# plumer/pbrs

Measured on AMD Instinct MI355X. Metric: Msamples/s, higher is better.
Workload: dtype f32

## Files before the change

### pbrs_amd/csrc/device/traverse.h

```cpp
#pragma once
#include "shapes.h"

#include "probes.h"

struct RaySpace {
    f3 o, d;
    f3 nr;
    bool fast;
};
PD uint32_t dir_in_range(float x) {
    uint32_t e = (pn_bits(x) >> 23) & 0xffu;
    return (e - (127u - 40u) <= 80u) ? 1u : 0u;
}
PD uint32_t origin_in_range(float x) {
    uint32_t u = pn_bits(x) & 0x7fffffffu;
    uint32_t e = u >> 23;
    return ((u == 0u) | (e - (127u - 60u) <= 100u)) ? 1u : 0u;
}
PD RaySpace make_space(f3 o, f3 d, bool scene_ok) {
    RaySpace r;
    r.o = o;
    r.d = d;
    r.fast = ((scene_ok ? 1u : 0u) & dir_in_range(d.x) & dir_in_range(d.y) & dir_in_range(d.z) & origin_in_range(o.x) &
              origin_in_range(o.y) & origin_in_range(o.z)) != 0u;
    r.nr = gray(0.0f);
    if (r.fast) r.nr = mk3(-(1.0f / d.x), -(1.0f / d.y), -(1.0f / d.z));
    return r;
}
PD RaySpace reload_world(const DevScene& S, LaneStack stk) {
    const float4 a = stk.ro[stk.item], b = stk.rd[stk.item];
    return make_space(mk3(a.x, a.y, a.z), mk3(b.x, b.y, b.z), S.fast_slab != 0);
}
#define PBRS_SPACE_WORLD 0u
#define PBRS_SPACE_MOVED 1u
#define PBRS_SPACE_TRANSLATED 2u
PD void leave_instance(const DevScene& S, LaneStack stk, uint32_t moved, RaySpace& C) {
    if (moved == PBRS_SPACE_TRANSLATED && C.fast) {
        const float4 a = stk.ro[stk.item];
        C.o = mk3(a.x, a.y, a.z);
    } else if (moved != PBRS_SPACE_WORLD) {
        C = reload_world(S, stk);
    }
}
PD float qdiv(float nn, float d, float nr) {
    const float q0 = nn * nr;
    const float e = __builtin_fmaf(d, q0, nn);
    return __builtin_fmaf(e, nr, q0);
}
PD bool slab_rs(const pbrs_node& n, const RaySpace& R, float t_max) {
    if (!R.fast) return slab_test(nmin(n), nmax(n), R.o, R.d, t_max);
    float t0x = qdiv(R.o.x - n.min[0], R.d.x, R.nr.x), t0y = qdiv(R.o.y - n.min[1], R.d.y, R.nr.y), t0z = qdiv(R.o.z - n.min[2], R.d.z, R.nr.z);
    float t1x = qdiv(R.o.x - n.max[0], R.d.x, R.nr.x), t1y = qdiv(R.o.y - n.max[1], R.d.y, R.nr.y), t1z = qdiv(R.o.z - n.max[2], R.d.z, R.nr.z);
    float lo_el = __builtin_fmaxf(__builtin_fmaxf(__builtin_fminf(t0x, t1x), __builtin_fminf(t0y, t1y)), __builtin_fminf(t0z, t1z));
    float hi_el = __builtin_fminf(__builtin_fminf(__builtin_fmaxf(t0x, t1x), __builtin_fmaxf(t0y, t1y)), __builtin_fmaxf(t0z, t1z));
    float t_low = __builtin_fmaxf(lo_el, 0.0f);
    float t_high = __builtin_fminf(hi_el, t_max);
    return t_low <= t_high;
}
#include "wide.h"

struct InstHead {
    uint32_t flags, blas_root, mesh_flags, wide_root;
};
static_assert(offsetof(pbrs_instance, flags) == 108 && offsetof(pbrs_instance, blas_root) == 112 && offsetof(pbrs_instance, mesh_flags) == 116 &&
                  offsetof(pbrs_instance, pad) == 120 && sizeof(pbrs_instance) == 128 && alignof(pbrs_instance) <= 16,
              "pbrs_instance layout (load_inst_head, wide root in pad[1], shading class in pad[0])");
static_assert(sizeof(pbrs_node) == 32 && offsetof(pbrs_node, a) == 12 && offsetof(pbrs_node, max) == 16 && offsetof(pbrs_node, b) == 28, "pbrs_node layout (load_node)");
static_assert(sizeof(pbrs_wnode) == 128 && offsetof(pbrs_wnode, hi) == 48 && offsetof(pbrs_wnode, child) == 96, "pbrs_wnode layout (wide_test)");
static_assert(sizeof(pbrs_tri_verts) == 48, "pbrs_tri_verts layout (load_tri)");
PD InstHead load_inst_head(const pbrs_instance& in) {
    uint32_t f = in.flags;
    uint4 r = *reinterpret_cast<const uint4*>(&in.blas_root);
    asm volatile("" : "+v"(f), "+v"(r.x), "+v"(r.y), "+v"(r.w));
    return {f, r.x, r.y, r.w};
}
PD uint32_t enter_instance(const DevScene& S, const pbrs_instance& in, uint32_t in_flags, RaySpace& C, bool need_slab, LaneStack stk) {
    if ((in_flags & PBRS_INSTANCE_IDENTITY) && C.fast && C.o.x != 0.0f && C.o.y != 0.0f && C.o.z != 0.0f) return PBRS_SPACE_WORLD;
    f3 oo = xf_apply(in.inv, C.o, 1.0f);
    if (need_slab && (in_flags & PBRS_INSTANCE_TRANSLATION) && C.fast) {
        C.o = oo;
        if (!(origin_in_range(oo.x) & origin_in_range(oo.y) & origin_in_range(oo.z))) {
            C.fast = false;
            C.nr = gray(0.0f);
        }
        return PBRS_SPACE_TRANSLATED;
    }
    f3 od = xf_apply(in.inv, C.d, 0.0f);
    if (need_slab) {
        C = make_space(oo, od, S.fast_slab != 0);
    } else {
        C.o = oo;
        C.d = od;
        C.fast = false;
    }
    return PBRS_SPACE_MOVED;
}

#ifndef PBRS_EARLY_OUT
#define PBRS_EARLY_OUT 1
#endif
#define PBRS_WALK_IDLE 0u
#define PBRS_WALK_NODE 1u
#define PBRS_WALK_LEAF 2u
#define PBRS_WALK_DONE 3u
#define PBRS_WALK_SCAN 5u
#define PBRS_WALK_XFER 4u

PD uint32_t lane_prefix(uint64_t mask) {
    return __builtin_amdgcn_mbcnt_hi((uint32_t)(mask >> 32), __builtin_amdgcn_mbcnt_lo((uint32_t)mask, 0u));
}
struct TriShare {
    uint32_t tag;
    uint32_t cnt;
    uint64_t has[4];
    uint32_t off[4];

    PD void build(uint32_t want) {
        const uint32_t lane = threadIdx.x & 63u;
        uint32_t o = 0;
        tag = 0;
        cnt = 0;
#pragma unroll
        for (uint32_t j = 0; j < 4u; ++j) {
            const uint64_t m = __ballot(want > j);
            has[j] = m;
            off[j] = o;
            if (m == 0) continue;
            const uint32_t p = o + lane_prefix(m);
            const bool send = want > j && p < 63u;
            tag |= (uint32_t)__builtin_amdgcn_ds_permute((int)((send ? p : 63u) << 2), send ? (int)(lane | j << 8 | 0x10000u) : 0);
            cnt += send ? 1u : 0u;
            o += (uint32_t)__popcll(m);
        }
    }
    PD bool helper() const { return tag != 0u; }
    PD uint32_t k() const { return (tag >> 8) & 3u; }
    PD uint32_t pos(uint32_t j) const { return off[j] + lane_prefix(has[j]); }
    PD uint32_t from_owner(uint32_t v) const { return (uint32_t)__builtin_amdgcn_ds_bpermute((int)(tag << 2), (int)v); }
    PD float from_owner(float v) const { return __uint_as_float(from_owner(__float_as_uint(v))); }
    PD f3 from_owner(f3 v) const { return mk3(from_owner(v.x), from_owner(v.y), from_owner(v.z)); }
    PD float from_helper(uint32_t at, float v) const {
        return __uint_as_float((uint32_t)__builtin_amdgcn_ds_bpermute((int)(at << 2), (int)__float_as_uint(v)));
    }
};

struct FlatScan {
    PD static uint32_t pull(uint32_t from, uint32_t v) { return (uint32_t)__builtin_amdgcn_ds_bpermute((int)(from << 2), (int)v); }
    PD static float pull(uint32_t from, float v) { return __uint_as_float(pull(from, __float_as_uint(v))); }
    struct Exact {
        RaySpace O;
        float t;
        PD Exact(const RaySpace& R, float t_max) : O(R), t(t_max) {}
        PD Exact from(uint32_t owner) const {
            Exact y = *this;
            y.O.o = mk3(pull(owner, O.o.x), pull(owner, O.o.y), pull(owner, O.o.z));
            y.O.d = mk3(pull(owner, O.d.x), pull(owner, O.d.y), pull(owner, O.d.z));
            y.O.nr = mk3(pull(owner, O.nr.x), pull(owner, O.nr.y), pull(owner, O.nr.z));
            y.O.fast = true;
            y.t = pull(owner, t);
            return y;
        }
        PD bool test(const pbrs_node& n) const { return slab_rs(n, O, t); }
    };
    struct Filter {
        f3 o, r;
        PD Filter(const RaySpace& R, float) : o(R.o), r(-R.nr) {}
        PD Filter from(uint32_t owner) const {
            Filter y = *this;
            y.o = mk3(pull(owner, o.x), pull(owner, o.y), pull(owner, o.z));
            y.r = mk3(pull(owner, r.x), pull(owner, r.y), pull(owner, r.z));
            return y;
        }
        PD bool test(const pbrs_node& n) const {
            return pn_slab_filter(r.x > 0.0f ? n.min[0] : n.max[0], r.y > 0.0f ? n.min[1] : n.max[1], r.z > 0.0f ? n.min[2] : n.max[2],
                                  r.x > 0.0f ? n.max[0] : n.min[0], r.y > 0.0f ? n.max[1] : n.min[1], r.z > 0.0f ? n.max[2] : n.min[2], o.x, o.y, o.z,
                                  r.x, r.y, r.z, pn_inf()) != 0;
        }
    };
    template <class Ray>
    PD static uint32_t scan(const DevScene& S, bool fresh, const RaySpace& R, float t_max, uint32_t& tested) {
        const uint64_t m = __ballot(fresh);
        if (m == 0) return 0u;
// ... 7 lines not shown
        uint32_t mine = 0;
        for (uint32_t base = 0; base < total; base += 64u) {
            const uint32_t p = base + lane;
            const bool valid = p < total;
            const uint32_t r = (p * magic) >> 16, h = p - r * H;
            const Ray O = mine_ray.from(pull(r, list));
            bool pass0 = false, pass1 = false;
            if (valid) {
                pass0 = O.test(load_node(S.nodes + S.flat_off + h));
                tested += 1u;
                if (h + H < S.n_flat) {
                    pass1 = O.test(load_node(S.nodes + S.flat_off + h + H));
                    tested += 1u;
                }
            }
            const uint64_t w0 = __ballot(pass0), w1 = __ballot(pass1);
            const int sft = (int)(rank * H) - (int)base;
            if (fresh && sft > -(int)H && sft < 64) {
                const uint64_t a = sft >= 0 ? w0 >> sft : w0 << -sft, b = sft >= 0 ? w1 >> sft : w1 << -sft;
                const uint32_t keep = (1u << H) - 1u;
                mine |= ((uint32_t)a & keep) | (((uint32_t)b & keep) << H);
            }
        }
        return mine;
    }
    PD static uint32_t run(const DevScene& S, bool fresh, const RaySpace& R, float t_max, uint32_t& tested) { return scan<Exact>(S, fresh, R, t_max, tested); }
    PD static uint32_t run_filter(const DevScene& S, bool fresh, const RaySpace& R, uint32_t& tested) { return scan<Filter>(S, fresh, R, pn_inf(), tested); }
};

template <bool STATS, uint32_t FEAT>
struct ClosestWalk {
    RaySpace C;
    Hit best;
    float t_max, lt, mt, mb1, mb2;
    uint32_t mprim, cur_inst;
    uint32_t inst_info;
    uint32_t leaf_a, leaf_end;
    int sp, blas_base;
    uint32_t cand;
    bool in_blas, moved;
    uint32_t mode;
    static constexpr bool EXT = (FEAT & PBRS_FEAT_EXTENT) != 0u;
    float win;
    bool win_has;
    PBRS_TP_FIELDS

    PD void start(const DevScene& S, f3 o, f3 d, float tmax, LaneStack stk) {
        C = make_space(o, d, S.fast_slab != 0);
        win = 0.0f;
        win_has = false;
        moved = false;
        best.t = pn_inf();
        best.inst = 0xffffffffu;
        best.prim = 0;
        best.b1 = best.b2 = 0.0f;
        in_blas = false;
        t_max = tmax;
        lt = tmax;
        mt = pn_inf();
        mprim = cur_inst = inst_info = leaf_a = leaf_end = 0;
        mb1 = mb2 = 0.0f;
        blas_base = 0;
        cand = 0;
        if ((FEAT & PBRS_FEAT_FLAT_TLAS) && !EXT && S.n_flat != 0u && C.fast) {
            sp = 0;
            mode = PBRS_WALK_SCAN;
        } else {
            stk.put(0, 0u);
            sp = 1;
            mode = PBRS_WALK_NODE;
        }
    }
    PD void scan_wave(const DevScene& S, Cnt<STATS>& cnt) {
        if (!(FEAT & PBRS_FEAT_FLAT_TLAS) || EXT) return;
        uint32_t tested = 0;
        const uint32_t mine = FlatScan::run_filter(S, mode == PBRS_WALK_SCAN, C, tested);
        if (STATS) cnt.c.tlas_nodes += tested;
        if (mode == PBRS_WALK_SCAN) {
            cand = mine;
            mode = PBRS_WALK_NODE;
        }
    }

    PD void node_step(const DevScene& S, LaneStack stk, Cnt<STATS>& cnt) {
        PBRS_TP(0);
        if (in_blas && sp == blas_base) {
            mode = exit_mode();
            return;
        }
        uint32_t ni;
        if (sp == 0) {
            if (!(FEAT & PBRS_FEAT_FLAT_TLAS) || cand == 0u) {
                mode = PBRS_WALK_DONE;
                return;
            }
            ni = S.flat_off + (uint32_t)__builtin_ctz(cand);
            cand &= cand - 1u;
        } else {
            ni = stk.get(--sp);
            if constexpr (EXT) {
                if (!in_blas && (ni & 0x80000000u)) {
                    const bool below_has = (ni & 0x40000000u) != 0u;
                    const float below = __uint_as_float(stk.get(--sp));
                    ni &= 0x3fffffffu;
                    if (win_has) t_max = win;
                    if (below_has && (!win_has || below < win)) win = below;
                    win_has = win_has || below_has;
                    lt = t_max;
                }
            }
            if (STATS) {
                if (in_blas) CNT(blas_nodes);
                else CNT(tlas_nodes);
            }
        }
        const pbrs_node node = walk_node<FEAT>(S, ni);
        PBRS_TP(1);
        if (!slab_rs(node, C, lt)) {
            PBRS_TP(2);
            if (PBRS_EARLY_OUT && in_blas && sp == blas_base) mode = exit_mode();
            return;
        }
        if (!(node.b & PBRS_LEAF_FLAG)) {
            bool left_first = !in_blas || comp(C.d, (int)(node.b & 3u)) > 0.0f;
            uint32_t left = ni + 1, right = node.a;
            if constexpr (EXT) {
                if (!in_blas) {
                    stk.put(sp++, __float_as_uint(win));
                    right |= 0x80000000u | (win_has ? 0x40000000u : 0u);
                    win_has = false;
                }
            }
            stk.put(sp++, left_first ? right : left);
            stk.put(sp++, left_first ? left : right);
            lt = in_blas ? mt : lt;
        } else if (in_blas) {
            PBRS_TP(3);
            PBRS_TP(4);
            leaf_a = node.a;
            leaf_end = node.a + (node.b & ~PBRS_LEAF_FLAG);
            if (leaf_end != leaf_a) mode = PBRS_WALK_LEAF;
            else lt = mt;
        } else {
            cur_inst = node.a;
            inst_info = (node.b >> PBRS_TLAS_LEAF_KIND_SHIFT) & 7u;
            mode = PBRS_WALK_XFER;
        }
    }

    PD void node_step_fast(const DevScene& S, LaneStack stk, Cnt<STATS>& cnt) {
        if constexpr (EXT) return;
        if (sp == (in_blas ? blas_base : 0) || !C.fast) return;
        PBRS_TP(0);
        const uint32_t ni = stk.get(--sp);
        if (STATS) {
            if (in_blas) CNT(blas_nodes);
            else CNT(tlas_nodes);
        }
        const pbrs_node node = walk_node<FEAT>(S, ni);
        PBRS_TP(1);
        RaySpace F = C;
        F.fast = true;
        if (!slab_rs(node, F, lt)) {
            PBRS_TP(2);
            return;
        }
        if (!(node.b & PBRS_LEAF_FLAG)) {
            bool left_first = !in_blas || comp(C.d, (int)(node.b & 3u)) > 0.0f;
            uint32_t left = ni + 1, right = node.a;
            stk.put(sp++, left_first ? right : left);
            stk.put(sp++, left_first ? left : right);
            lt = in_blas ? mt : lt;
        } else if (in_blas) {
            PBRS_TP(3);
            PBRS_TP(4);
            leaf_a = node.a;
            leaf_end = node.a + (node.b & ~PBRS_LEAF_FLAG);
            if (leaf_end != leaf_a) mode = PBRS_WALK_LEAF;
            else lt = mt;
        } else {
            cur_inst = node.a;
            inst_info = (node.b >> PBRS_TLAS_LEAF_KIND_SHIFT) & 7u;
            mode = PBRS_WALK_XFER;
        }
    }

    PD void meet_best(Cnt<STATS>& cnt) {
        if (mt < pn_inf() || (inst_info & 0x80000000u)) {
            CNT(instance_hits);
            if constexpr (EXT) {
                if (!win_has || !(win < mt)) win = mt;
                win_has = true;
            }
            if (!(best.t < mt)) {
                best.t = mt;
                best.inst = cur_inst;
                best.prim = mprim;
                best.b1 = mb1;
                best.b2 = mb2;
                if constexpr (!EXT) t_max = mt;
            }
        }
    }
    PD uint32_t exit_mode() const {
        const bool nothing_above = blas_base == 0 && (!(FEAT & PBRS_FEAT_FLAT_TLAS) || cand == 0u);
        return nothing_above ? PBRS_WALK_DONE : PBRS_WALK_XFER;
    }
    PD void finish(Cnt<STATS>& cnt) {
        if (in_blas) {
            in_blas = false;
            meet_best(cnt);
        }
    }
    PD void xfer_step(const DevScene& S, LaneStack stk, Cnt<STATS>& cnt) {
        mode = PBRS_WALK_NODE;
        if (in_blas) {
            PBRS_TP(7);
            in_blas = false;
            leave_instance(S, stk, !moved ? PBRS_SPACE_WORLD : (inst_info & 0x40000000u) ? PBRS_SPACE_TRANSLATED : PBRS_SPACE_MOVED, C);
            meet_best(cnt);
            lt = t_max;
            return;
        }
        const pbrs_instance& in = S.inst[cur_inst];
        CNT(instances);
        PBRS_TP(6);
        const uint32_t kind = inst_info;
        if ((FEAT & PBRS_FEAT_ANALYTIC) && kind != PBRS_SHAPE_MESH && kind != PBRS_SHAPE_TRIANGLE) {
            analytic_visit(S, in, kind, cnt);
            return;
        }
        const InstHead H = load_inst_head(in);
        const uint32_t space = enter_instance(S, in, H.flags, C, kind == PBRS_SHAPE_MESH, stk);
        moved = space != PBRS_SPACE_WORLD;
        in_blas = true;
        blas_base = sp;
        lt = t_max;
        mt = pn_inf();
        if (kind == PBRS_SHAPE_MESH) {
            inst_info = kind | (H.mesh_flags << 3) | (space == PBRS_SPACE_TRANSLATED ? 0x40000000u : 0u);
            stk.put(sp++, H.blas_root);
        } else if (kind == PBRS_SHAPE_TRIANGLE) {
            inst_info = kind | (PBRS_MESH_SHADING_OK_MASK << 3);
            leaf_a = H.blas_root;
            leaf_end = H.blas_root + 1u;
            mode = PBRS_WALK_LEAF;
        }
    }

    PD void analytic_visit(const DevScene& S, const pbrs_instance& in, uint32_t kind, Cnt<STATS>& cnt) {
        if (!(FEAT & PBRS_FEAT_ANALYTIC)) return;
        const f3 o = xf_apply(in.inv, C.o, 1.0f), d = xf_apply(in.inv, C.d, 0.0f);
        const float ext = t_max;
        const float* p = S.shapes[in.shape_index].p;
// ... 505 lines not shown
```

### pbrs_amd/csrc/host/scene_prepare.cpp

```cpp
#include "scene_prepare.h"

#include <algorithm>
#include <cstring>
#include <map>
#include <string>

#include "../../../include/pbrs_numeric.h"
#include "../../../include/pbrs_scene_spec.h"

namespace pbrs {
namespace {

SceneCheck refuse(int code, const char* message) { return SceneCheck{code, message, SceneLevels{}}; }

void tree_heights(const pbrs_node* nodes, uint32_t n, std::vector<uint32_t>& h) {
    h.assign(n, 1u);
    for (uint32_t i = n; i-- > 0;)
        if (!(nodes[i].b & PBRS_LEAF_FLAG)) h[i] = std::max(h[i + 1], h[nodes[i].a]) + 1u;
}

SceneLevels scene_levels(const pbrs_scene_desc& d) {
    SceneLevels l;
    std::vector<uint32_t> th, bh;
    tree_heights(d.tlas_nodes, d.n_tlas_nodes, th);
    tree_heights(d.blas_nodes, d.n_blas_nodes, bh);
    l.tlas = th[0];
    for (uint32_t i = 0; i < d.n_meshes; ++i) l.max_blas = std::max(l.max_blas, bh[d.meshes[i].root]);
    for (uint32_t i = 0; i < d.n_instances; ++i)
        if (d.instances[i].shape_kind == PBRS_SHAPE_MESH) l.max_blas = std::max(l.max_blas, bh[d.instances[i].blas_root]);
    l.stack = std::max(l.tlas, l.tlas - 1u + l.max_blas);
    bool has_quad = false, has_mesh = false;
    for (uint32_t i = 0; i < d.n_instances; ++i) {
        has_quad = has_quad || d.instances[i].shape_kind == PBRS_SHAPE_QUAD;
        has_mesh = has_mesh || d.instances[i].shape_kind == PBRS_SHAPE_MESH;
    }
    l.exact_extent = has_quad && has_mesh;
    if (l.exact_extent) l.stack += l.tlas + 1u;
    return l;
}

bool tlas_scanned(const pbrs_scene_desc& d) { return d.n_instances >= PBRS_FLAT_TLAS_MIN && d.n_instances <= PBRS_FLAT_TLAS_MAX_ANYHIT; }

uint32_t build_wide(const std::vector<pbrs_node>& nodes, uint32_t x, std::vector<pbrs_wnode>& out, uint32_t level, uint32_t& levels) {
    const uint32_t me = (uint32_t)out.size();
    out.push_back(pbrs_wnode{});
    levels = std::max(levels, level + 1u);
    uint32_t slot_node[4] = {0, 0, 0, 0};
    uint32_t used = 0, info = nodes[x].b & 3u;
    const uint32_t child[2] = {x + 1u, nodes[x].a};
    for (uint32_t s = 0; s < 2; ++s) {
        const pbrs_node& ch = nodes[child[s]];
        if (ch.b & PBRS_LEAF_FLAG) {
            slot_node[2 * s] = child[s];
            used |= 1u << (2 * s);
        } else {
            info |= (ch.b & 3u) << (2 + 2 * s);
            slot_node[2 * s] = child[s] + 1u;
            slot_node[2 * s + 1] = ch.a;
            used |= 3u << (2 * s);
        }
    }
    pbrs_wnode w{};
    for (uint32_t k = 0; k < 4; ++k) {
        w.child[k] = PBRS_WREF_NONE;
        if (!((used >> k) & 1u)) {
            for (int a = 0; a < 3; ++a) w.lo[a][k] = PBRS_WIDE_UNUSED_PLANE, w.hi[a][k] = -PBRS_WIDE_UNUSED_PLANE;
            continue;
        }
        const pbrs_node& n = nodes[slot_node[k]];
        for (int a = 0; a < 3; ++a) {
            w.lo[a][k] = n.min[a];
            w.hi[a][k] = n.max[a];
        }
        w.child[k] = (n.b & PBRS_LEAF_FLAG) ? (PBRS_WREF_LEAF | slot_node[k]) : build_wide(nodes, slot_node[k], out, level + 1u, levels);
    }
    w.child[0] |= (info & 15u) << PBRS_WREF_AXIS_SHIFT;
    w.child[2] |= ((info >> 4) & 3u) << PBRS_WREF_AXIS_SHIFT;
    out[me] = w;
    return me;
}

}

SceneCheck check_scene(const pbrs_scene_desc& d) {
    if (d.n_tlas_nodes == 0 || d.n_instances == 0) return refuse(PBRS_E_INVALID, "scene without instances");
    for (uint32_t i = 0; i < d.n_tlas_nodes; ++i) {
        const pbrs_node& n = d.tlas_nodes[i];
        if (n.b & PBRS_LEAF_FLAG) {
            if (n.a >= d.n_instances) return refuse(PBRS_E_INVALID, "tlas leaf references a missing instance");
        } else if (n.a >= d.n_tlas_nodes || i + 1 >= d.n_tlas_nodes) {
            return refuse(PBRS_E_INVALID, "tlas child out of range");
        } else if (n.a <= i) {
            return refuse(PBRS_E_INVALID, "tlas nodes are not in pre-order");
        }
    }
    for (uint32_t i = 0; i < d.n_blas_nodes; ++i) {
        const pbrs_node& n = d.blas_nodes[i];
        if (n.b & PBRS_LEAF_FLAG) {
            uint32_t cnt = n.b & ~PBRS_LEAF_FLAG;
            if ((uint64_t)n.a + cnt > d.n_triangles) return refuse(PBRS_E_INVALID, "blas leaf range out of range");
        } else if (n.a >= d.n_blas_nodes || i + 1 >= d.n_blas_nodes || (n.b & 3u) > 2u) {
            return refuse(PBRS_E_INVALID, "blas child out of range");
        } else if (n.a <= i) {
            return refuse(PBRS_E_INVALID, "blas nodes are not in pre-order");
        }
    }
    for (uint32_t i = 0; i < d.n_meshes; ++i)
        if (d.meshes[i].root >= d.n_blas_nodes) return refuse(PBRS_E_INVALID, "mesh root out of range");
    for (uint32_t i = 0; i < d.n_instances; ++i) {
        const pbrs_instance& in = d.instances[i];
        if (in.material >= d.n_materials) return refuse(PBRS_E_INVALID, "instance material out of range");
        if (in.shape_kind > PBRS_SHAPE_MESH) return refuse(PBRS_E_INVALID, "unknown shape kind");
        if (in.shape_kind == PBRS_SHAPE_MESH ? in.shape_index >= d.n_meshes : in.shape_index >= d.n_shapes)
            return refuse(PBRS_E_INVALID, "instance shape out of range");
        if (in.shape_kind == PBRS_SHAPE_MESH ? in.blas_root >= d.n_blas_nodes : (in.shape_kind == PBRS_SHAPE_TRIANGLE && in.blas_root >= d.n_triangles))
            return refuse(PBRS_E_INVALID, "instance blas_root out of range");
    }
    for (uint32_t i = 0; i < d.n_materials; ++i) {
        const pbrs_material& m = d.materials[i];
        if (m.n_bxdfs > PBRS_MAX_BXDFS || (uint64_t)m.first_bxdf + m.n_bxdfs > d.n_bxdfs) return refuse(PBRS_E_INVALID, "material lobes out of range");
        if (m.vis_bxdf > d.n_bxdfs) return refuse(PBRS_E_INVALID, "material visualiser record out of range");
    }
    for (uint32_t i = 0; i < d.n_bxdfs; ++i) {
        const uint32_t t = d.bxdfs[i].tex & ~PBRS_BXDF_TEX_DROP_IF_BLACK;
        if (t > d.n_textures) return refuse(PBRS_E_INVALID, "lobe texture out of range");
        if (d.bxdfs[i].kind > PBRS_BXDF_FOURIER) return refuse(PBRS_E_INVALID, "unknown lobe kind");
        if (d.bxdfs[i].kind == PBRS_BXDF_FOURIER && d.bxdfs[i].intrusion >= d.n_fourier_tables) return refuse(PBRS_E_INVALID, "Fourier lobe table out of range");
    }
    for (uint32_t i = 0; i < d.n_fourier_tables; ++i) {
        const pbrs_fourier_table& t = d.fourier_tables[i];
        const uint64_t n = t.n_mu, nn = n * n, nf = d.n_tex_floats, nw = d.n_tex_words;
        if (n < 3 || (t.n_channels != 1 && t.n_channels != 3)) return refuse(PBRS_E_INVALID, "Fourier table: sizes");
        if (t.mu + n > nf || t.cdf + nn > nf || t.a0 + nn > nf || (uint64_t)t.a + t.n_coeffs > nf || (uint64_t)t.recip + t.m_max > nf ||
            t.a_offset + nn > nw || t.m_lookup + nn > nw)
            return refuse(PBRS_E_INVALID, "Fourier table: arrays out of range");
        for (uint64_t k = 0; k < n; ++k) {
            const float m0 = d.tex_floats[t.mu + k];
            if (!pn_isfinite(m0) || (k + 1 < n && !(m0 < d.tex_floats[t.mu + k + 1]))) return refuse(PBRS_E_INVALID, "Fourier table: mu is not finite and strictly ascending");
        }
        for (uint64_t k = 0; k < nn; ++k) {
            const uint64_t off = d.tex_words[t.a_offset + k], len = d.tex_words[t.m_lookup + k];
            if (len > t.m_max || off + len * t.n_channels > t.n_coeffs) return refuse(PBRS_E_INVALID, "Fourier table: series out of range");
        }
    }
    for (uint32_t i = 0; i < d.n_textures; ++i) {
        const pbrs_texture& t = d.textures[i];
        if (t.kind == PBRS_TEX_PERLIN) {
            if ((uint64_t)t.data + 768 > d.n_tex_floats || (uint64_t)t.perm + 768 > d.n_tex_words) return refuse(PBRS_E_INVALID, "perlin tables out of range");
            for (uint32_t k = 0; k < 768; ++k)
                if (d.tex_words[t.perm + k] > 255u) return refuse(PBRS_E_INVALID, "perlin permutation entry above 255");
        } else if (t.kind == PBRS_TEX_IMAGE) {
            if (t.width == 0 || t.height == 0 || (uint64_t)t.data + 3ull * t.width * t.height > d.n_tex_floats)
                return refuse(PBRS_E_INVALID, "image texels out of range");
        } else if (t.kind != PBRS_TEX_CHECKER) {
            return refuse(PBRS_E_INVALID, "unknown texture kind");
        }
    }
    if (d.env_kind > PBRS_ENV_DUSK) return refuse(PBRS_E_INVALID, "unknown environment kind");
    if (d.env_kind == PBRS_ENV_IMAGE && (d.env_texture >= d.n_textures || d.textures[d.env_texture].kind != PBRS_TEX_IMAGE))
        return refuse(PBRS_E_INVALID, "environment map is not an image texture");
    for (uint32_t i = 0; i < d.n_area_lights; ++i) {
        uint32_t k = d.area_lights[i].shape_kind;
        if (!(k == PBRS_SHAPE_SPHERE || k == PBRS_SHAPE_DISK || k == PBRS_SHAPE_TRIANGLE || k == PBRS_SHAPE_QUAD))
            return refuse(PBRS_E_INVALID, "area light shape kind");
    }
    const SceneLevels levels = scene_levels(d);
    if ((size_t)levels.stack * kBlock * sizeof(uint32_t) > kLdsBytesPerCU / 2) return refuse(PBRS_E_LIMIT, "traversal stack exceeds the LDS budget");
    uint64_t n_nodes = (uint64_t)d.n_tlas_nodes;
    if (tlas_scanned(d))
        for (uint32_t i = 0; i < d.n_tlas_nodes; ++i) n_nodes += (d.tlas_nodes[i].b & PBRS_LEAF_FLAG) ? 1u : 0u;
    if (n_nodes + d.n_blas_nodes > 0x7fffffffull) return refuse(PBRS_E_LIMIT, "too many BVH nodes");
    if ((n_nodes + d.n_blas_nodes) * sizeof(pbrs_node) >= (1ull << 32)) return refuse(PBRS_E_LIMIT, "too many BVH nodes (the walks address them with 32-bit byte offsets)");
    return SceneCheck{PBRS_OK, nullptr, levels};
}

PreparedScene prepare_scene(const pbrs_scene_desc& d, const SceneLevels& lv, const DevOverrides& dev) {
    PreparedScene P;
    DevScene& S = P.S;
    SceneFacts& f = P.facts;
    P.stack_depth = lv.stack;
    {
        auto coord_ok = [](float b) {
            uint32_t u = pn_bits(b) & 0x7fffffffu, e = u >> 23;
            return u == 0u || (e >= 127u - 60u && e <= 127u + 40u);
        };
        bool ok = true;
        for (uint32_t i = 0; i < d.n_tlas_nodes && ok; ++i)
            for (int a = 0; a < 3; ++a) ok = ok && coord_ok(d.tlas_nodes[i].min[a]) && coord_ok(d.tlas_nodes[i].max[a]);
        for (uint32_t i = 0; i < d.n_blas_nodes && ok; ++i)
            for (int a = 0; a < 3; ++a) ok = ok && coord_ok(d.blas_nodes[i].min[a]) && coord_ok(d.blas_nodes[i].max[a]);
        S.fast_slab = ok ? 1u : 0u;
    }
    S.exact_extent = lv.exact_extent ? 1u : 0u;

    const bool scan = tlas_scanned(d);
    std::vector<pbrs_node>& nodes = P.nodes;
    nodes.assign(d.tlas_nodes, d.tlas_nodes + d.n_tlas_nodes);
    S.flat_off = (uint32_t)nodes.size();
    if (scan)
        for (uint32_t i = 0; i < d.n_tlas_nodes; ++i)
            if (d.tlas_nodes[i].b & PBRS_LEAF_FLAG) nodes.push_back(d.tlas_nodes[i]);
    S.n_flat = (uint32_t)nodes.size() - S.flat_off;
    const uint64_t blas_off = nodes.size();
    nodes.insert(nodes.end(), d.blas_nodes, d.blas_nodes + d.n_blas_nodes);
    for (size_t i = blas_off; i < nodes.size(); ++i)
        if (!(nodes[i].b & PBRS_LEAF_FLAG)) nodes[i].a += (uint32_t)blas_off;
    P.walk_bytes = nodes.size() * sizeof(pbrs_node) + (uint64_t)d.n_triangles * sizeof(pbrs_tri_verts) + (uint64_t)d.n_instances * sizeof(pbrs_instance);

    std::vector<pbrs_instance>& inst = P.inst;
    inst.assign(d.instances, d.instances + d.n_instances);
    std::vector<uint32_t> mat_class(d.n_materials, 0u);
    {
        std::vector<std::string> sigs;
        for (uint32_t m = 0; m < d.n_materials; ++m) {
            const pbrs_material& mt = d.materials[m];
            if (mt.n_bxdfs == 0) continue;
            std::string sig;
            for (uint32_t k = 0; k < mt.n_bxdfs; ++k) {
                const pbrs_bxdf& bx = d.bxdfs[mt.first_bxdf + k];
                sig += (char)('a' + bx.kind);
                sig += (char)('a' + (bx.kind == PBRS_BXDF_SPECULAR ? bx.intrusion : 0u));
                sig += (char)('a' + (bx.kind == PBRS_BXDF_DIFFUSE ? bx.oren_nayar : bx.fresnel));
                sig += (char)('a' + (bx.kind == PBRS_BXDF_MICROFACET && bx.alpha_x != bx.alpha_y ? 1 : 0));
                sig += bx.tex ? 't' : '-';
            }
            size_t at = 0;
            while (at < sigs.size() && sigs[at] != sig) ++at;
            if (at == sigs.size()) sigs.push_back(sig);
            mat_class[m] = (uint32_t)std::min<size_t>(at + 1, PBRS_MAX_CLASSES - 1);
        }
        S.n_classes = (uint32_t)std::min<size_t>(sigs.size(), PBRS_MAX_CLASSES - 1);
        const std::string lam_sig = {(char)('a' + PBRS_BXDF_DIFFUSE), 'a', 'a', 'a', '-'};
        for (size_t at = 0; at < sigs.size() && at + 1 < PBRS_MAX_CLASSES - 1; ++at)
            if (sigs[at] == lam_sig) f.lambert_class = (uint32_t)at + 1;
        const std::string fou_sig = {(char)('a' + PBRS_BXDF_FOURIER), 'a', 'a', 'a', '-'};
        for (size_t at = 0; at < sigs.size() && at + 1 < PBRS_MAX_CLASSES - 1; ++at)
            if (sigs[at] == fou_sig) f.fourier_class = (uint32_t)at + 1;
    }
    for (pbrs_instance& in : inst) {
        in.pad[0] = mat_class[in.material];
        if (in.shape_kind == PBRS_SHAPE_MESH) in.blas_root += (uint32_t)blas_off;
        bool linear_identity = true;
        for (int r = 0; r < 3; ++r)
            for (int k = 0; k < 3; ++k) linear_identity = linear_identity && pn_bits(in.inv[r][k]) == pn_bits(r == k ? 1.0f : 0.0f);
        in.flags &= ~PBRS_INSTANCE_TRANSLATION;
        if (linear_identity) in.flags |= PBRS_INSTANCE_TRANSLATION;
    }
    for (pbrs_instance& in : inst) in.pad[1] = PBRS_WREF_NONE;
    S.wide_cap = 4u;
    if (scan && S.fast_slab != 0u) {
        std::vector<pbrs_wnode>& wide = P.wide;
        std::map<uint32_t, uint32_t> wide_of_root;
        uint32_t levels = 0;
        for (pbrs_instance& in : inst) {
            if (in.shape_kind != PBRS_SHAPE_MESH || (nodes[in.blas_root].b & PBRS_LEAF_FLAG)) continue;
            auto it = wide_of_root.find(in.blas_root);
            if (it == wide_of_root.end()) it = wide_of_root.emplace(in.blas_root, build_wide(nodes, in.blas_root, wide, 0u, levels)).first;
            in.pad[1] = it->second;
        }
        if (levels >= PBRS_WIDE_MIN_LEVELS && wide.size() * sizeof(pbrs_wnode) < (1ull << 32)) {
            P.walk_bytes += wide.size() * sizeof(pbrs_wnode);
            S.wide_cap = std::max(4u, std::min(3u * levels + 1u, (uint32_t)PBRS_WIDE_STACK_MAX));
            P.wide_levels = levels;
        } else {
            wide.clear();
            for (pbrs_instance& in : inst) in.pad[1] = PBRS_WREF_NONE;
        }
    }

    S.n_area = d.n_area_lights;
    S.n_delta = d.n_delta_lights;
    S.env_kind = d.env_kind;
    S.env_texture = d.env_texture;
    std::memcpy(S.env_scale, d.env_scale, sizeof S.env_scale);
    std::memcpy(S.env, d.env_constant, sizeof S.env);
    S.has_env = (d.env_kind != PBRS_ENV_CONSTANT || !(S.env[0] <= 0.0f && S.env[1] <= 0.0f && S.env[2] <= 0.0f)) ? 1u : 0u;
    S.refill_below = lv.max_blas >= PBRS_LONG_WALK_HEIGHT ? PBRS_REFILL_BELOW_LONG : PBRS_REFILL_BELOW_SHORT;
    S.refill_below_shadow = lv.max_blas >= PBRS_LONG_WALK_HEIGHT ? PBRS_REFILL_BELOW_LONG_SHADOW : PBRS_REFILL_BELOW_SHORT;
    if (dev.refill_below) S.refill_below = S.refill_below_shadow = *dev.refill_below;
    f.long_walks = (S.n_flat ? 0u : lv.tlas) + lv.max_blas >= PBRS_LONG_WALK_HEIGHT;
    f.full_steps = S.fast_slab == 0u;
    f.tlas_scanned = S.n_flat != 0u;
    S.features = (S.n_flat != 0u && d.n_instances <= PBRS_FLAT_TLAS_MAX) ? PBRS_FEAT_FLAT_TLAS : 0u;
    f.wide_ok = S.fast_slab != 0u && P.wide_levels >= PBRS_WIDE_MIN_LEVELS;
    for (uint32_t i = 0; i < d.n_instances; ++i) {
        const pbrs_instance& in = d.instances[i];
        if (in.shape_kind == PBRS_SHAPE_MESH) {
            if (!(in.mesh_flags & PBRS_MESH_SHADING_OK_MASK)) S.features |= PBRS_FEAT_SHADING_CHECK;
        } else if (in.shape_kind != PBRS_SHAPE_TRIANGLE) {
// ... 44 lines not shown
```

### pbrs_amd/csrc/host/scene_prepare.h

```cpp
#pragma once
#include <cstdint>
#include <vector>

#include "../device/scene.h"
#include "kernel_choice.h"

namespace pbrs {

struct SceneLevels {
    uint32_t tlas = 0;
    uint32_t max_blas = 0;
    uint32_t stack = 0;
    bool exact_extent = false;
};
struct SceneCheck {
    int code = PBRS_OK;
    const char* message = nullptr;
    SceneLevels levels;
};
SceneCheck check_scene(const pbrs_scene_desc& d);

struct PreparedScene {
    DevScene S{};
    std::vector<pbrs_node> nodes;
    std::vector<pbrs_instance> inst;
    std::vector<pbrs_wnode> wide;
    uint32_t wide_levels = 0;
    SceneFacts facts;
    uint32_t stack_depth = 0;
    bool has_vis_records = false;
    uint64_t walk_bytes = 0;
};
PreparedScene prepare_scene(const pbrs_scene_desc& d, const SceneLevels& levels, const DevOverrides& dev);

}
```

### pbrs_amd/csrc/pbrs_gpu.hip

```cpp
#include <hip/hip_runtime.h>

#include <algorithm>
#include <cmath>
#include <cstdio>
#include <cstdlib>
#include <cstring>
#include <utility>
#include <mutex>
#include <optional>
#include <string>
#include <vector>

#include "../../include/pbrs_gpu.h"
#include "device/kernels.h"
#include "host/scene_prepare.h"
#include "host/arg_checks.h"
#include "host/pass_plan.h"
#include "device/aov.h"
#include "device/film.h"
#include "device/denoise.h"
#include "device/moments.h"
#include "device/matte.h"
#include "device/passes.h"
#include "device/temporal.h"
// ... 866 lines not shown
    c->overlap_passes = c->dev.overlap_passes;
    for (int k = 0; ok && k < 2; ++k) {
        hipEvent_t ev = nullptr;
        ok = hipEventCreate(&ev) == hipSuccess;
        if (ok) c->total_ev.push_back(ev);
    }
    for (pbrs_ctx::PassSet& set : c->pass_set) ok = ok && hipMalloc(reinterpret_cast<void**>(&set.counters), kCounters.words * sizeof(uint32_t)) == hipSuccess;
    ok = ok && hipMalloc(reinterpret_cast<void**>(&c->gcnt), 2 * sizeof(GlobalCounters)) == hipSuccess &&
         hipMalloc(reinterpret_cast<void**>(&c->nonfinite), sizeof(unsigned long long)) == hipSuccess &&
         hipMalloc(reinterpret_cast<void**>(&c->bounce_acc), (2 * PBRS_STATS_MAX_BOUNCES + 2) * sizeof(unsigned long long)) == hipSuccess &&
         hipMemset(c->bounce_acc, 0, (2 * PBRS_STATS_MAX_BOUNCES + 2) * sizeof(unsigned long long)) == hipSuccess &&
         hipMemset(c->nonfinite, 0, sizeof(unsigned long long)) == hipSuccess &&
         hipHostMalloc(reinterpret_cast<void**>(&c->split_host), 2 * sizeof(unsigned long long), hipHostMallocDefault) == hipSuccess &&
         hipEventCreateWithFlags(&c->split_ev, hipEventDisableTiming) == hipSuccess;
    ok = ok && configure_kernels(c) == PBRS_OK;
    if (!ok) {
        pbrs_destroy(c);
        return PBRS_E_DEVICE;
    }
    *out = c;
    return PBRS_OK;
}

void pbrs_destroy(pbrs_ctx* c) {
    if (!c) return;
    (void)hipSetDevice(c->device);
    if (c->stream) (void)hipStreamSynchronize(c->stream);
    if (c->second_stream) (void)hipStreamSynchronize(c->second_stream);
    free_scene(c);
    free_work(c);
    for (DeviceBuffer& b : c->buf)
        if (b.p) (void)hipFree(b.p);
    for (pbrs_ctx::PassSet& set : c->pass_set)
        if (set.counters) (void)hipFree(set.counters);
    for (int k = 0; k < 2; ++k)
        if (c->pass_set[k].accumulated) (void)hipEventDestroy(c->pass_set[k].accumulated);
    for (int k = 0; k < 2; ++k)
        if (c->pass_set[k].late) (void)hipEventDestroy(c->pass_set[k].late);
    if (c->second_stream) (void)hipStreamDestroy(c->second_stream);
    if (c->gcnt) (void)hipFree(c->gcnt);
    if (c->nonfinite) (void)hipFree(c->nonfinite);
    if (c->bounce_acc) (void)hipFree(c->bounce_acc);
    if (c->split_host) (void)hipHostFree(c->split_host);
    if (c->split_ev) (void)hipEventDestroy(c->split_ev);
    for (auto& e : c->events) {
        (void)hipEventDestroy(e.a);
        (void)hipEventDestroy(e.b);
    }
    for (auto& e : c->total_ev) (void)hipEventDestroy(e);
    if (c->own_stream) (void)hipStreamDestroy(c->own_stream);
    delete c;
}

const char* pbrs_last_error(const pbrs_ctx* c) { return c ? c->error.c_str() : "null context"; }

int pbrs_set_stream(pbrs_ctx* c, void* hip_stream) {
    if (!c) return PBRS_E_INVALID;
    c->main_stream = hip_stream ? static_cast<hipStream_t>(hip_stream) : c->own_stream;
    c->stream = c->main_stream;
    return PBRS_OK;
}

int pbrs_set_pass_overlap(pbrs_ctx* c, int enabled) {
    if (!c) return PBRS_E_INVALID;
    c->overlap_passes = enabled != 0;
    return PBRS_OK;
}

int pbrs_upload_scene(pbrs_ctx* c, const pbrs_scene_desc* d) {
    if (!c || !d) return PBRS_E_INVALID;
    HIPCHK(c, hipSetDevice(c->device));
    const SceneCheck chk = check_scene(*d);
    if (chk.code != PBRS_OK) return fail(c, chk.code, chk.message);
    PreparedScene P = prepare_scene(*d, chk.levels, c->dev);
    const KernelChoice choice = choose_kernels(P.facts, c->dev);
    KernelPlan plan;
    if (!bind_kernels(choice, plan)) return fail(c, PBRS_E_DEVICE, "no kernel instantiation for this scene's feature set");
    (void)hipStreamSynchronize(c->stream);
    (void)hipStreamSynchronize(c->second_stream);
    free_scene(c);
    c->plan = plan;
    DevScene S = P.S;
    int rc;
    if ((rc = upload(c, P.nodes.data(), P.nodes.size(), &S.nodes))) return rc;
    if (!P.wide.empty() && (rc = upload(c, P.wide.data(), P.wide.size(), &S.wnodes))) return rc;
    if ((rc = upload(c, P.inst.data(), P.inst.size(), &S.inst))) return rc;
    if ((rc = upload(c, d->shapes, d->n_shapes, &S.shapes))) return rc;
    if ((rc = upload(c, d->meshes, d->n_meshes, &S.meshes))) return rc;
    if ((rc = upload(c, d->tri_verts, d->n_triangles, &S.tv))) return rc;
    if ((rc = upload(c, d->tri_shade, d->n_triangles, &S.ts))) return rc;
    if ((rc = upload(c, d->materials, d->n_materials, &S.mats))) return rc;
    if ((rc = upload(c, d->bxdfs, d->n_bxdfs, &S.bxdfs))) return rc;
    if ((rc = upload(c, d->area_lights, d->n_area_lights, &S.alights))) return rc;
    if ((rc = upload(c, d->delta_lights, d->n_delta_lights, &S.dlights))) return rc;
    if ((rc = upload(c, d->textures, d->n_textures, &S.textures))) return rc;
    if ((rc = upload(c, d->tex_floats, d->n_tex_floats, &S.tex_floats))) return rc;
    if ((rc = upload(c, d->tex_words, d->n_tex_words, &S.tex_words))) return rc;
    if ((rc = upload(c, d->fourier_tables, d->n_fourier_tables, &S.fourier))) return rc;
    const bool lds_scene = choice.lds_staging == PBRS_FEAT_LDS_SCENE;
    S.lds_off_words = P.stack_depth * kBlock;
    S.lds_nodes = lds_scene ? (uint32_t)P.nodes.size() : choice.lds_staging == PBRS_FEAT_LDS_TOP ? d->n_tlas_nodes : 0u;
    S.lds_tris = lds_scene ? d->n_triangles : 0u;
    S.lds_inst = lds_scene ? d->n_instances : 0u;
    S.lds_shapes = lds_scene ? d->n_shapes : 0u;
    c->S = S;
    c->overlap_from = c->dev.overlap_from.value_or(P.walk_bytes <= (4ull << 20) ? 2u : 4u);
    c->has_vis_records = P.has_vis_records;
    c->stack_depth = P.stack_depth;
    c->has_scene = true;
    c->split_decision = 0;
    c->split_probe_in_flight = false;
    return PBRS_OK;
}

int pbrs_render_tile_passes_device(pbrs_ctx* c, const pbrs_camera* cam, const pbrs_render_params* p, float* rgb_out_device,
                                   const pbrs_aov_buffers* aovs_device, float* variance_device, const pbrs_matte_params* params,
                                   const pbrs_matte_buffers* matte_device, const pbrs_pass_buffers* passes_device, pbrs_stats* stats_out) {
    if (!c) return PBRS_E_INVALID;
    if (!rgb_out_device) return fail(c, PBRS_E_INVALID, "null output");
    return render(c, cam, p, nullptr, make_targets(rgb_out_device, aovs_device, variance_device, params, matte_device, passes_device), false, stats_out);
}

int pbrs_render_tile_matte_device(pbrs_ctx* c, const pbrs_camera* cam, const pbrs_render_params* p, float* rgb_out_device,
                                  const pbrs_aov_buffers* aovs_device, float* variance_device, const pbrs_matte_params* params,
                                  const pbrs_matte_buffers* matte_device, pbrs_stats* stats_out) {
    return pbrs_render_tile_passes_device(c, cam, p, rgb_out_device, aovs_device, variance_device, params, matte_device, nullptr, stats_out);
}

int pbrs_render_tile_aovs_var_device(pbrs_ctx* c, const pbrs_camera* cam, const pbrs_render_params* p, float* rgb_out_device,
                                     const pbrs_aov_buffers* aovs_device, float* variance_device, pbrs_stats* stats_out) {
    return pbrs_render_tile_matte_device(c, cam, p, rgb_out_device, aovs_device, variance_device, nullptr, nullptr, stats_out);
}

int pbrs_render_tile_aovs_device(pbrs_ctx* c, const pbrs_camera* cam, const pbrs_render_params* p, float* rgb_out_device, const pbrs_aov_buffers* aovs_device,
                                 pbrs_stats* stats_out) {
    return pbrs_render_tile_matte_device(c, cam, p, rgb_out_device, aovs_device, nullptr, nullptr, nullptr, stats_out);
}

int pbrs_render_tile_device(pbrs_ctx* c, const pbrs_camera* cam, const pbrs_render_params* p, float* rgb_out_device, pbrs_stats* stats_out) {
    return pbrs_render_tile_matte_device(c, cam, p, rgb_out_device, nullptr, nullptr, nullptr, nullptr, stats_out);
}

int pbrs_render_tile_passes(pbrs_ctx* c, const pbrs_camera* cam, const pbrs_render_params* p, float* rgb_out_host, const pbrs_aov_buffers* aovs_host,
                            float* variance_host, const pbrs_matte_params* params, const pbrs_matte_buffers* matte_host, const pbrs_pass_buffers* passes_host,
                            pbrs_stats* stats_out) {
    if (!c) return PBRS_E_INVALID;
    if (!rgb_out_host) return fail(c, PBRS_E_INVALID, "null output");
    return render(c, cam, p, nullptr, make_targets(rgb_out_host, aovs_host, variance_host, params, matte_host, passes_host), true, stats_out);
}

int pbrs_render_tile_matte(pbrs_ctx* c, const pbrs_camera* cam, const pbrs_render_params* p, float* rgb_out_host, const pbrs_aov_buffers* aovs_host,
                           float* variance_host, const pbrs_matte_params* params, const pbrs_matte_buffers* matte_host, pbrs_stats* stats_out) {
    return pbrs_render_tile_passes(c, cam, p, rgb_out_host, aovs_host, variance_host, params, matte_host, nullptr, stats_out);
}

int pbrs_render_tile_aovs_var(pbrs_ctx* c, const pbrs_camera* cam, const pbrs_render_params* p, float* rgb_out_host, const pbrs_aov_buffers* aovs_host,
                              float* variance_host, pbrs_stats* stats_out) {
    return pbrs_render_tile_matte(c, cam, p, rgb_out_host, aovs_host, variance_host, nullptr, nullptr, stats_out);
}

int pbrs_render_tile_aovs(pbrs_ctx* c, const pbrs_camera* cam, const pbrs_render_params* p, float* rgb_out_host, const pbrs_aov_buffers* aovs_host,
                          pbrs_stats* stats_out) {
    return pbrs_render_tile_matte(c, cam, p, rgb_out_host, aovs_host, nullptr, nullptr, nullptr, stats_out);
}

int pbrs_render_tile(pbrs_ctx* c, const pbrs_camera* cam, const pbrs_render_params* p, float* rgb_out_host, pbrs_stats* stats_out) {
// ... 666 lines not shown
```

Measured before the change: 1584.

## Cull BVH children using quantized split planes packed into node flags

Precomputes, per interior BLAS node, quantized positions of the left child's max and right child's min along the split axis and packs them into spare bits of the node's b field. During traversal, the ray's entry/exit interval from the parent slab test is compared against these planes so that children the ray cannot reach are not pushed. This is meant to avoid stack pushes, node fetches and slab tests for unreachable children. It adds extra ALU per interior node and relies on the b field's bits 2-29 being unused by other decoders.

```diff
diff --git a/pbrs_amd/csrc/device/split_planes.h b/pbrs_amd/csrc/device/split_planes.h
--- /dev/null
+++ b/pbrs_amd/csrc/device/split_planes.h
@@ -0,0 +1,20 @@
+#pragma once
+#include <stdint.h>
+
+#if defined(__HIPCC__)
+#define PBRS_SP_FN __host__ __device__ static inline
+#else
+#define PBRS_SP_FN static inline
+#endif
+
+#define PBRS_PLANE_BITS 14u
+#define PBRS_PLANE_MAX ((1u << PBRS_PLANE_BITS) - 1u)
+#define PBRS_PLANE_DOWN_SHIFT 2u
+#define PBRS_PLANE_UP_SHIFT 16u
+
+PBRS_SP_FN float pbrs_plane_step(float lo, float hi) { return (hi - lo) * 0x1p-14f; }
+PBRS_SP_FN float pbrs_plane_down(uint32_t q, float step, float lo) { return __builtin_fmaf((float)q, step, lo); }
+PBRS_SP_FN float pbrs_plane_up(uint32_t q, float step, float hi) { return __builtin_fmaf(-(float)q, step, hi); }
+PBRS_SP_FN uint32_t pbrs_plane_qd(uint32_t b) { return (b >> PBRS_PLANE_DOWN_SHIFT) & PBRS_PLANE_MAX; }
+PBRS_SP_FN uint32_t pbrs_plane_qu(uint32_t b) { return (b >> PBRS_PLANE_UP_SHIFT) & PBRS_PLANE_MAX; }
+PBRS_SP_FN uint32_t pbrs_plane_pack(uint32_t qd, uint32_t qu) { return qd << PBRS_PLANE_DOWN_SHIFT | qu << PBRS_PLANE_UP_SHIFT; }
diff --git a/pbrs_amd/csrc/device/traverse.h b/pbrs_amd/csrc/device/traverse.h
--- a/pbrs_amd/csrc/device/traverse.h
+++ b/pbrs_amd/csrc/device/traverse.h
@@ -47,16 +47,21 @@
     const float e = __builtin_fmaf(d, q0, nn);
     return __builtin_fmaf(e, nr, q0);
 }
-PD bool slab_rs(const pbrs_node& n, const RaySpace& R, float t_max) {
+PD bool slab_rs(const pbrs_node& n, const RaySpace& R, float t_max, float& t_low, float& hi_el) {
     if (!R.fast) return slab_test(nmin(n), nmax(n), R.o, R.d, t_max);
     float t0x = qdiv(R.o.x - n.min[0], R.d.x, R.nr.x), t0y = qdiv(R.o.y - n.min[1], R.d.y, R.nr.y), t0z = qdiv(R.o.z - n.min[2], R.d.z, R.nr.z);
     float t1x = qdiv(R.o.x - n.max[0], R.d.x, R.nr.x), t1y = qdiv(R.o.y - n.max[1], R.d.y, R.nr.y), t1z = qdiv(R.o.z - n.max[2], R.d.z, R.nr.z);
     float lo_el = __builtin_fmaxf(__builtin_fmaxf(__builtin_fminf(t0x, t1x), __builtin_fminf(t0y, t1y)), __builtin_fminf(t0z, t1z));
-    float hi_el = __builtin_fminf(__builtin_fminf(__builtin_fmaxf(t0x, t1x), __builtin_fmaxf(t0y, t1y)), __builtin_fmaxf(t0z, t1z));
-    float t_low = __builtin_fmaxf(lo_el, 0.0f);
+    hi_el = __builtin_fminf(__builtin_fminf(__builtin_fmaxf(t0x, t1x), __builtin_fmaxf(t0y, t1y)), __builtin_fmaxf(t0z, t1z));
+    t_low = __builtin_fmaxf(lo_el, 0.0f);
     float t_high = __builtin_fminf(hi_el, t_max);
     return t_low <= t_high;
 }
+PD bool slab_rs(const pbrs_node& n, const RaySpace& R, float t_max) {
+    float t_low = 0.0f, hi_el = 0.0f;
+    return slab_rs(n, R, t_max, t_low, hi_el);
+}
+#include "split_planes.h"
 #include "wide.h"
 
 struct InstHead {
@@ -98,6 +103,9 @@
 
 #ifndef PBRS_EARLY_OUT
 #define PBRS_EARLY_OUT 1
+#endif
+#ifndef PBRS_SPLIT_PLANE_CULL
+#define PBRS_SPLIT_PLANE_CULL 1
 #endif
 #define PBRS_WALK_IDLE 0u
 #define PBRS_WALK_NODE 1u
@@ -271,6 +279,31 @@
         }
     }
 
+    static constexpr bool CULL = PBRS_SPLIT_PLANE_CULL != 0 && !STATS && !EXT && !(FEAT & PBRS_FEAT_LDS_TOP);
+    PD uint32_t cull_children(const pbrs_node& X, float dk, float t_low, float hi_el) const {
+        const int k = (int)(X.b & 3u);
+        const float lo = comp(nmin(X), k), hi = comp(nmax(X), k);
+        const float step = pbrs_plane_step(lo, hi);
+        const float pd = pbrs_plane_down(pbrs_plane_qd(X.b), step, lo), pu = pbrs_plane_up(pbrs_plane_qu(X.b), step, hi);
+        const bool pos = dk > 0.0f;
+        const float ok = comp(C.o, k), nrk = comp(C.nr, k);
+        const float e_near = qdiv(ok - (pos ? pu : pd), dk, nrk), e_far = qdiv(ok - (pos ? pd : pu), dk, nrk);
+        const float T = __builtin_fminf(hi_el, mt);
+        return (e_near < t_low ? 0u : 1u) | (e_far > T ? 0u : 2u);
+    }
+    PD void push_children(LaneStack stk, bool left_first, uint32_t left, uint32_t right, uint32_t keep) {
+        const uint32_t far = left_first ? right : left, near = left_first ? left : right;
+        if constexpr (!CULL) {
+            stk.put(sp++, far);
+            stk.put(sp++, near);
+        } else {
+            stk.put(sp, far);
+            sp += (int)(keep >> 1);
+            stk.put(sp, near);
+            sp += (int)(keep & 1u);
+        }
+    }
+
     PD void node_step(const DevScene& S, LaneStack stk, Cnt<STATS>& cnt) {
         PBRS_TP(0);
         if (in_blas && sp == blas_base) {
@@ -305,13 +338,15 @@
         }
         const pbrs_node node = walk_node<FEAT>(S, ni);
         PBRS_TP(1);
-        if (!slab_rs(node, C, lt)) {
+        float t_low = 0.0f, hi_el = 0.0f;
+        if (!slab_rs(node, C, lt, t_low, hi_el)) {
             PBRS_TP(2);
             if (PBRS_EARLY_OUT && in_blas && sp == blas_base) mode = exit_mode();
             return;
         }
         if (!(node.b & PBRS_LEAF_FLAG)) {
-            bool left_first = !in_blas || comp(C.d, (int)(node.b & 3u)) > 0.0f;
+            const float dk = comp(C.d, (int)(node.b & 3u));
+            bool left_first = !in_blas || dk > 0.0f;
             uint32_t left = ni + 1, right = node.a;
             if constexpr (EXT) {
                 if (!in_blas) {
@@ -320,8 +355,11 @@
                     win_has = false;
                 }
             }
-            stk.put(sp++, left_first ? right : left);
-            stk.put(sp++, left_first ? left : right);
+            uint32_t keep = 3u;
+            if constexpr (CULL) {
+                if (in_blas && C.fast) keep = cull_children(node, dk, t_low, hi_el);
+            }
+            push_children(stk, left_first, left, right, keep);
             lt = in_blas ? mt : lt;
         } else if (in_blas) {
             PBRS_TP(3);
@@ -350,15 +388,20 @@
         PBRS_TP(1);
         RaySpace F = C;
         F.fast = true;
-        if (!slab_rs(node, F, lt)) {
+        float t_low = 0.0f, hi_el = 0.0f;
+        if (!slab_rs(node, F, lt, t_low, hi_el)) {
             PBRS_TP(2);
             return;
         }
         if (!(node.b & PBRS_LEAF_FLAG)) {
-            bool left_first = !in_blas || comp(C.d, (int)(node.b & 3u)) > 0.0f;
+            const float dk = comp(C.d, (int)(node.b & 3u));
+            bool left_first = !in_blas || dk > 0.0f;
             uint32_t left = ni + 1, right = node.a;
-            stk.put(sp++, left_first ? right : left);
-            stk.put(sp++, left_first ? left : right);
+            uint32_t keep = 3u;
+            if constexpr (CULL) {
+                if (in_blas) keep = cull_children(node, dk, t_low, hi_el);
+            }
+            push_children(stk, left_first, left, right, keep);
             lt = in_blas ? mt : lt;
         } else if (in_blas) {
             PBRS_TP(3);
diff --git a/pbrs_amd/csrc/host/scene_prepare.cpp b/pbrs_amd/csrc/host/scene_prepare.cpp
--- a/pbrs_amd/csrc/host/scene_prepare.cpp
+++ b/pbrs_amd/csrc/host/scene_prepare.cpp
@@ -7,6 +7,7 @@
 
 #include "../../../include/pbrs_numeric.h"
 #include "../../../include/pbrs_scene_spec.h"
+#include "../device/split_planes.h"
 
 namespace pbrs {
 namespace {
@@ -80,6 +81,30 @@
     return me;
 }
 
+bool coord_ok(float b) {
+    const uint32_t u = pn_bits(b) & 0x7fffffffu, e = u >> 23;
+    return u == 0u || (e >= 127u - 60u && e <= 127u + 40u);
+}
+
+uint32_t split_planes(const std::vector<pbrs_node>& nodes, uint32_t x) {
+    const pbrs_node &X = nodes[x], &L = nodes[x + 1u], &R = nodes[X.a];
+    for (int a = 0; a < 3; ++a) {
+        const bool inside = X.min[a] <= L.min[a] && L.min[a] <= L.max[a] && L.max[a] <= X.max[a] && X.min[a] <= R.min[a] && R.min[a] <= R.max[a] && R.max[a] <= X.max[a];
+        if (!inside) return 0u;
+    }
+    const uint32_t k = X.b & 3u;
+    const float lo = X.min[k], hi = X.max[k], step = pbrs_plane_step(lo, hi);
+    if (!(step > 0.0f) || !pn_isfinite(step)) return 0u;
+    uint32_t qd = 0u, qu = 0u;
+    for (uint32_t bit = 1u << (PBRS_PLANE_BITS - 1u); bit; bit >>= 1) {
+        if (pbrs_plane_down(qd | bit, step, lo) <= R.min[k]) qd |= bit;
+        if (pbrs_plane_up(qu | bit, step, hi) >= L.max[k]) qu |= bit;
+    }
+    if (!coord_ok(pbrs_plane_down(qd, step, lo))) qd = 0u;
+    if (!coord_ok(pbrs_plane_up(qu, step, hi))) qu = 0u;
+    return pbrs_plane_pack(qd, qu);
+}
+
 }
 
 SceneCheck check_scene(const pbrs_scene_desc& d) {
@@ -180,10 +205,6 @@
     SceneFacts& f = P.facts;
     P.stack_depth = lv.stack;
     {
-        auto coord_ok = [](float b) {
-            uint32_t u = pn_bits(b) & 0x7fffffffu, e = u >> 23;
-            return u == 0u || (e >= 127u - 60u && e <= 127u + 40u);
-        };
         bool ok = true;
         for (uint32_t i = 0; i < d.n_tlas_nodes && ok; ++i)
             for (int a = 0; a < 3; ++a) ok = ok && coord_ok(d.tlas_nodes[i].min[a]) && coord_ok(d.tlas_nodes[i].max[a]);
@@ -205,6 +226,10 @@
     nodes.insert(nodes.end(), d.blas_nodes, d.blas_nodes + d.n_blas_nodes);
     for (size_t i = blas_off; i < nodes.size(); ++i)
         if (!(nodes[i].b & PBRS_LEAF_FLAG)) nodes[i].a += (uint32_t)blas_off;
+    P.node_planes.assign(nodes.size(), 0u);
+    if (S.fast_slab != 0u)
+        for (size_t i = blas_off; i < nodes.size(); ++i)
+            if (!(nodes[i].b & PBRS_LEAF_FLAG)) P.node_planes[i] = split_planes(nodes, (uint32_t)i);
     P.walk_bytes = nodes.size() * sizeof(pbrs_node) + (uint64_t)d.n_triangles * sizeof(pbrs_tri_verts) + (uint64_t)d.n_instances * sizeof(pbrs_instance);
 
     std::vector<pbrs_instance>& inst = P.inst;
diff --git a/pbrs_amd/csrc/host/scene_prepare.h b/pbrs_amd/csrc/host/scene_prepare.h
--- a/pbrs_amd/csrc/host/scene_prepare.h
+++ b/pbrs_amd/csrc/host/scene_prepare.h
@@ -23,6 +23,7 @@
 struct PreparedScene {
     DevScene S{};
     std::vector<pbrs_node> nodes;
+    std::vector<uint32_t> node_planes;
     std::vector<pbrs_instance> inst;
     std::vector<pbrs_wnode> wide;
     uint32_t wide_levels = 0;
diff --git a/pbrs_amd/csrc/pbrs_gpu.hip b/pbrs_amd/csrc/pbrs_gpu.hip
--- a/pbrs_amd/csrc/pbrs_gpu.hip
+++ b/pbrs_amd/csrc/pbrs_gpu.hip
@@ -972,6 +972,7 @@
     c->plan = plan;
     DevScene S = P.S;
     int rc;
+    for (size_t i = 0; i < P.nodes.size(); ++i) P.nodes[i].b |= P.node_planes[i];
     if ((rc = upload(c, P.nodes.data(), P.nodes.size(), &S.nodes))) return rc;
     if (!P.wide.empty() && (rc = upload(c, P.wide.data(), P.wide.size(), &S.wnodes))) return rc;
     if ((rc = upload(c, P.inst.data(), P.inst.size(), &S.inst))) return rc;
```

Result: faster. 1686 (median of 6 runs) (+6.4%).
